# tomwhite/disq

Hardware: AMD Instinct MI355X
Metric: decompressed BAM GB/s + reads/sec (whole node) at 1/2/4/8 MI355X (higher is better)
Workload: dtype u8

## Files before the change

### disq_amd/csrc/dq_inflate3.hip

```cpp
#include "dq_inflate_core.h"
#include "dq_internal.h"

#include <mutex>
#include <vector>

namespace dq {
namespace {

using namespace dqi;

#define DQ_HD __device__ __host__ __attribute__((always_inline)) inline

#ifndef DQ_BLK_WG
#define DQ_BLK_WG 512
#endif
constexpr int WG = DQ_BLK_WG;
static_assert(WG % 128 == 0 && WG >= 512 && WG <= 1024, "whole waves on every SIMD");
constexpr int NWV = WG / 64;
constexpr int NDEC = WG;
constexpr uint32_t OV_DEFAULT = 96;
#ifndef DQ_TAIL_OV
#define DQ_TAIL_OV OV_DEFAULT
#endif
constexpr int OUTCAP = 65536 + 24;
#ifndef DQ_CSTEP
#define DQ_CSTEP 0
#endif
#ifndef DQ_RES_NB
#define DQ_RES_NB (WG == 512 ? 4 : 2)
#endif
#ifndef DQ_RES_G
#define DQ_RES_G 1
#endif
constexpr int RES_NXT = DQ_RES_NB * DQ_RES_G * WG;
constexpr int NCARRY = (65536 + RES_NXT - 1) / RES_NXT + 1;


constexpr int LR = 10, DR = 8;
constexpr int LSB = 15 - LR, DSB = 15 - DR;
constexpr int LSLOTS = 16, DSLOTS = 4;
constexpr int MAXGRP = 64;
constexpr int T_LSUB = 1 << LR;
constexpr int T_DROOT = T_LSUB + LSLOTS * (1 << LSB);
constexpr int T_DSUB = T_DROOT + (1 << DR);
constexpr int T_END = T_DSUB + DSLOTS * (1 << DSB);
constexpr int HB_WORDS = 160;
constexpr uint16_t E_SLOW = 0x0080;
constexpr uint32_t LL_EOB = 0xF810, LL_BAD = 0xF910;
DQ_HD uint16_t ent_ll(uint32_t sym, uint32_t len) {
  if (sym < 256) return (uint16_t)(sym << 8 | len);
  if (sym == 256) return (uint16_t)(LL_EOB | len);
  if (sym > 285) return (uint16_t)(LL_BAD | len);
  const uint32_t k = sym - 257;
  const uint32_t x = (k < 8 || k == 28) ? 0u : (k - 4) >> 2;
  const uint32_t base = k < 8 ? k + 3 : k == 28 ? 258u : ((4u + (k & 3u)) << ((k - 4) >> 2)) + 3u;
  return (uint16_t)((base - 3) << 8 | x << 5 | 16u | len);
}
DQ_HD uint16_t ent_d(uint32_t d, uint32_t len) {
  if (d >= 30) return (uint16_t)(0x4000u | len);
  const uint32_t x = d < 4 ? 0u : (d - 2) >> 1;
  const uint32_t m = d < 2 ? d : 2u + (d & 1u), sh = d < 2 ? 0u : (d >> 1) - 1u;
  return (uint16_t)(m << 12 | sh << 8 | x << 4 | len);
}

enum : int32_t { F_EXIT = 0, F_EOB = 1, F_ERR = 2, F_END = 3 };

constexpr int TOUT = 4096;
constexpr int TAIL_MAX_BITS = 32768;
constexpr int TW = 4;
#ifndef DQ_ROOT_REG
#define DQ_ROOT_REG 1
#endif
#ifndef DQ_TAIL_HDR1
#define DQ_TAIL_HDR1 1
#endif
constexpr int T_NCK = 4;
#ifndef DQ_TAIL_SEG
#define DQ_TAIL_SEG 96
#endif
constexpr int TAIL_SEG_MIN = DQ_TAIL_SEG;
constexpr int TIM_W = 32;
struct TailDesc {
  int32_t pos;
  int32_t produced;
  uint32_t crc_raw;
  int32_t flag;
};

struct alignas(16) LdsI {
  static constexpr int kLSUB = T_LSUB, kDROOT = T_DROOT, kDSUB = T_DSUB;
  [[maybe_unused]] static constexpr int kTEND = T_END;
  static constexpr bool kPair = true;
  alignas(8) uint32_t bm[2048];
  union {
    struct {
      uint16_t T[T_END];
      HuffCanon hl, hd;
      uint16_t lend[16], dend[16];
      uint16_t lent[288];
      uint16_t dent[32];
      union {
        uint16_t pair[1 << LR];
        struct {
          uint8_t lens[320];
          uint8_t clen[20];
          uint16_t clt[128];
          union {
            struct {
              int32_t cntw[NWV];
              int32_t cnts[NWV];
              uint32_t ginfo[MAXGRP + 32];
              uint32_t cntp[8][8];
              uint16_t pref[320];
            };
            struct {
              uint8_t exitm[NWV][16];
              int32_t ent[NWV + 1];
              int32_t wt[NWV];
              int32_t lv[NWV];
              int32_t endp;
            };
          };
        } h;
      } x;
    } d;
    struct {
      uint16_t last_start[1024];
      uint16_t nxt[RES_NXT];
      int32_t carry_ms[NCARRY];
      uint32_t carry_desc[NCARRY];
    } r;
    uint32_t crc4[4][256];
  } u;
  int32_t misc[32];
  union {
    struct {
      int32_t wsum[16];
      int32_t small[8 * 7];
    };
    uint32_t scratch[16 + 8 * 7];
  };
  alignas(16) uint8_t out[OUTCAP];
};
static_assert(sizeof(((LdsI*)nullptr)->scratch) >= 64 * 4, "one emit dummy word per lane");
static_assert(offsetof(LdsI, out) < 65536 - 4096, "the tables' offsets fit the DS offset field");
static_assert(2 * sizeof(LdsI) <= 160 * 1024, "two workgroups per CU");
static_assert(HB_WORDS * 4 <= T_END * 2, "header staging fits the decode table");

__device__ inline uint32_t* emit_dummy(LdsI& L) { return L.scratch; }

__constant__ uint32_t c_crc4[4][256];
__constant__ uint32_t c_x2n[32];
__constant__ uint32_t c_x8n[TOUT + 1];
constexpr int CRC_SL = 4 * (((65536 / 4 + WG - 1) / WG) | 1);
static_assert(CRC_SL * WG >= 65536, "the slices cover the largest block");
__constant__ uint32_t c_slice_shift[WG];
__constant__ uint8_t c_clorder3[19] = {16, 17, 18, 0, 8, 7, 9, 6, 10, 5, 11, 4, 12, 3, 13, 2, 14, 1, 15};

enum { M_ERR = 0, M_SLOW = 1 , M_A = 4, M_LAST, M_MORE, M_MORE1,
       M_LQ0 = 15, M_LQN, M_DQ0, M_DQN, M_NEXT,
       M_LASTF, M_RCNT = 28 ,
       M_DIRTY = 30  };

template <class LT>
__device__ __attribute__((always_inline)) inline void set_err(LT& L, int32_t code) { atomicCAS(&L.misc[M_ERR], 0, code); }


#define DQ_AI __device__ __attribute__((always_inline)) inline

DQ_AI int tid_fresh() {
  int t = (int)threadIdx.x;
  asm volatile("" : "+v"(t));
  return t;
}

typedef uint32_t u32x4 __attribute__((ext_vector_type(4)));
DQ_AI void st_nt(uint4* d, uint4 v) {
  u32x4 x = {v.x, v.y, v.z, v.w};
  __builtin_nontemporal_store(x, reinterpret_cast<u32x4*>(d));
}

struct GSrc {
  const uint32_t* __restrict__ p;
#ifdef DQ_CHECKED
  uint32_t lim;
  uint32_t tag;
#endif
  DQ_AI uint32_t operator[](uint32_t i) const {
#ifdef DQ_CHECKED
    DQ_CHKV(i < lim, CHK_K2_BITS, tag | min(i - lim + 1, 4095u));
#endif
    return *reinterpret_cast<const uint32_t*>(reinterpret_cast<const uint8_t*>(p) + (i << 2));
  }
};

#ifndef DQ_BR64
#define DQ_BR64 0
#endif
#if DQ_BR64
struct BitR {
  uint64_t bb;
  uint32_t bc;
  uint32_t wp;
  uint32_t nw;
};
template <class S>
DQ_AI void br_init(BitR& r, const S& W, uint32_t bitpos) {
  const uint32_t wi = bitpos >> 5;
  const uint64_t lo = W[wi], hi = W[wi + 1];
  const uint32_t sh = bitpos & 31;
  r.bb = ((hi << 32) | lo) >> sh;
  r.bc = 64 - sh;
  r.wp = wi + 2;
  r.nw = W[r.wp];
}
template <class S>
DQ_AI void br_refill(BitR& r, const S& W) {
  const bool need = r.bc <= 32;
  r.bb |= (uint64_t)(need ? r.nw : 0u) << r.bc;
  r.bc += need ? 32u : 0u;
  r.wp += need ? 1u : 0u;
  r.nw = W[r.wp];
}
DQ_AI uint32_t br_pos(const BitR& r) { return r.wp * 32 - r.bc; }
DQ_AI uint32_t br_peek(const BitR& r) { return (uint32_t)r.bb; }
template <class S>
DQ_AI void br_take(BitR& r, const S&, uint32_t n) {
  r.bb >>= n;
  r.bc -= n;
}
#else
struct BitR {
  uint32_t p;
  uint32_t w0, w1;
  uint32_t nw;
};
template <class S>
DQ_AI void br_init(BitR& r, const S& W, uint32_t bitpos) {
  const uint32_t wi = bitpos >> 5;
  r.w0 = W[wi];
  r.w1 = W[wi + 1];
  r.nw = W[wi + 2];
  r.p = bitpos;
}
template <class S>
DQ_AI void br_refill(BitR&, const S&) {}
DQ_AI uint32_t br_pos(const BitR& r) { return r.p; }
DQ_AI uint32_t br_peek(const BitR& r) { return __builtin_amdgcn_alignbit(r.w1, r.w0, r.p); }
template <class S>
DQ_AI void br_take(BitR& r, const S& W, uint32_t n) {
  const uint32_t q = r.p + n;
  const bool c = (q ^ r.p) >= 32u;
  r.w0 = c ? r.w1 : r.w0;
  r.w1 = c ? r.nw : r.w1;
  r.p = q;
  r.nw = W[(q >> 5) + 2];
}
#endif
DQ_AI uint32_t peek_bits(const uint32_t* __restrict__ W, uint32_t pos, uint32_t n) {
  const uint32_t wi = pos >> 5;
  const uint64_t v = ((uint64_t)W[wi + 1] << 32) | W[wi];
  return (uint32_t)(v >> (pos & 31)) & ((1u << n) - 1);
}

template <class LT>
DQ_AI uint32_t load_desc(const LT& L, int a) {
  const uint32_t* w = reinterpret_cast<const uint32_t*>(L.out + (a & ~3));
  return __builtin_amdgcn_alignbyte(w[1], w[0], (uint32_t)a & 3u) & 0xffffffu;
}

DQ_AI uint32_t zx16(uint16_t v) {
#ifndef DQ_NO_ZX16
  uint32_t x = v;
  asm("" : "+v"(x));
  return x;
#else
  return v;
#endif
}

template <bool SLOW, class LT>
DQ_AI uint32_t ll_second(const LT& L, uint32_t e, uint32_t bb) {
  const uint32_t sb = (e >> 4) & 7;
  DQ_CHK(LT::kLSUB + (e >> 7) + ((bb >> LR) & ((1u << sb) - 1)) < (uint32_t)LT::kDROOT, CHK_K2_TABLE);
  if (!SLOW) return L.u.d.T[LT::kLSUB + (e >> 7) + ((bb >> LR) & ((1u << sb) - 1))];
  if (sb) return L.u.d.T[LT::kLSUB + (e >> 7) + ((bb >> LR) & ((1u << sb) - 1))];
  if (!(e & E_SLOW)) return 0u;
  int l = 0;
  const int k = canon_decode(bb, L.u.d.hl, LR + 1, &l);
  return k < 0 ? 0u : L.u.d.lent[k];
}
template <bool SLOW, class LT>
DQ_AI uint32_t d_second(const LT& L, uint32_t e, uint32_t bb) {
  const uint32_t sb = (e >> 4) & 7;
  DQ_CHK(LT::kDSUB + (e >> 7) + ((bb >> DR) & ((1u << sb) - 1)) < (uint32_t)LT::kTEND, CHK_K2_TABLE);
  if (!SLOW) return L.u.d.T[LT::kDSUB + (e >> 7) + ((bb >> DR) & ((1u << sb) - 1))];
  if (sb) return L.u.d.T[LT::kDSUB + (e >> 7) + ((bb >> DR) & ((1u << sb) - 1))];
  if (!(e & E_SLOW)) return 0u;
  int l = 0;
  const int k = canon_decode(bb, L.u.d.hd, DR + 1, &l);
  return k < 0 ? 0u : L.u.d.dent[k];
}


template <bool SLOW, class S, class LT>
DQ_AI bool dsym(BitR& r, const S& W, const LT& L, uint32_t p, uint32_t lim,
                uint32_t& len, uint32_t& dist, uint32_t& lit2, bool& is_m, uint32_t& e) {
  br_refill(r, W);
  uint32_t bb = br_peek(r);
  const uint32_t ri = bb & ((1u << LR) - 1);
  e = L.u.d.T[ri];
  uint32_t pe = 0;
  if constexpr (LT::kPair) pe = zx16(L.u.d.x.pair[ri]);
  if ((e & 15) == 0) e = ll_second<SLOW>(L, e, bb);
  const uint32_t nb = e & 15;
  const uint32_t lx = __builtin_amdgcn_ubfe(e, 5, 3);
  is_m = (e & 16) != 0;
  len = (e >> 8) + (is_m ? 3u : 0u) + __builtin_amdgcn_ubfe(bb, nb, lx);
  const bool two = pe != 0 && p + nb < lim;
  lit2 = two ? pe >> 8 : 0xffffffffu;
  br_take(r, W, nb + lx + (two ? (pe & 15) : 0u));
  br_refill(r, W);
  bb = br_peek(r);
  uint32_t e2 = zx16(L.u.d.T[LT::kDROOT + (bb & ((1u << DR) - 1))]);
  if (is_m && (e2 & 15) == 0) e2 = d_second<SLOW>(L, e2, bb);
  const uint32_t nb2 = e2 & 15, dx = __builtin_amdgcn_ubfe(e2, 4, 4);
  dist = (__builtin_amdgcn_ubfe(e2, 12, 2) << __builtin_amdgcn_ubfe(e2, 8, 4)) + 1u +
         __builtin_amdgcn_ubfe(bb, nb2, dx);
  br_take(r, W, is_m ? nb2 + dx : 0u);
  return (SLOW && nb == 0) || (e & 0xFEF0u) == 0xF810u ||
         (is_m && ((SLOW && nb2 == 0) || (e2 & 0x4000u)));
}
DQ_AI uint32_t stop_end(uint32_t e, uint32_t p) {
  return (e & 15) != 0 && (e & 0xFFF0u) == LL_EOB ? p + (e & 15) : 0xffffffffu;
}
// ... 620 lines not shown
    const int32_t bfinal = (int32_t)(h & 1), btype = (int32_t)((h >> 1) & 3);
    const int32_t herr = pos + 3 > endbits ? ST_OVERREAD : btype == 3 ? ST_BAD_BLOCKTYPE : 0;
    if (herr) {
      if (t == 0) L.misc[M_ERR] = herr;
      break;
    }
    if (btype == 0) {
      const uint32_t q = (pos + 3 + 7) & ~7u;
      const uint8_t* bp = reinterpret_cast<const uint8_t*>(W) + q / 8;
      const uint32_t len = bp[0] | ((uint32_t)bp[1] << 8), nl = bp[2] | ((uint32_t)bp[3] << 8);
      const int32_t serr = (len ^ 0xffffu) != nl ? ST_BAD_STORED : q + 32 + 8 * len > endbits ? ST_OVERREAD : 0;
      if (serr) {
        if (t == 0) L.misc[M_ERR] = serr;
        break;
      }
      const uint8_t* sp = bp + 4;
      const int32_t n = min((int32_t)len, isize - produced);
      DQ_CHK(sh + produced + n <= OUTCAP, CHK_K2_IMAGE);
      for (int i = t; i < n; i += WG) L.out[sh + produced + i] = sp[i];
      produced += n;
      pos = q + 32 + 8 * len;
      __syncthreads();
      if (bfinal) break;
      continue;
    }
    const int nlen = btype == 1 ? 288 : (int)((h >> 3) & 31) + 257;
    const int ndist = btype == 1 ? 32 : (int)((h >> 8) & 31) + 1;
    if (btype == 2 && (nlen > 286 || ndist > 30)) {
      if (t == 0) L.misc[M_ERR] = ST_BAD_TABLE;
      break;
    }
    if (btype == 1) {
      for (int i = t; i < 320; i += WG) L.u.d.x.h.lens[i] = fixed_len(i);
      if (t == 0) L.misc[M_A] = (int32_t)(pos + 3);
      __syncthreads();
    } else {
      const int ncode = (int)((h >> 13) & 15) + 4;
      for (int i = t; i < 320; i += WG) L.u.d.x.h.lens[i] = 0;
      if (t < HB_WORDS) reinterpret_cast<uint32_t*>(L.u.d.T)[t] = hw;
      if (t < 19) L.u.d.x.h.clen[c_clorder3[t]] = t < ncode ? (uint8_t)hcl : 0;
      __syncthreads();
      if (t < 128) {
        bool ok = true;
        L.u.d.x.h.clt[t] = clt_entry(L.u.d.x.h.clen, t, &ok);
        if (t == 0 && !ok) set_err(L, ST_BAD_TABLE);
      }
      __syncthreads();
      if (L.misc[M_ERR]) break;
      {
        const uint64_t tr0 = TIMING ? __builtin_amdgcn_s_memtime() : 0;
        const uint32_t a = read_lengths(L, clpos + 3 * (uint32_t)ncode, nlen, ndist, endbits, hbase);
        if (t == 0) L.misc[M_A] = (int32_t)a;
        if (TIMING && t == 0) tacc[8] += __builtin_amdgcn_s_memtime() - tr0;
      }
      __syncthreads();
      if (L.misc[M_ERR]) break;
      if (L.u.d.x.h.lens[256] == 0) {
        if (t == 0) L.misc[M_ERR] = ST_BAD_TABLE;
        break;
      }
    }
    TST(0);
    build_tables(L, nlen, ndist);
    if (TIMING && t == 0) tacc[11] += __builtin_amdgcn_s_memtime() - tlast;
    if (L.misc[M_ERR]) break;
    for (int i = t; i < (1 << LR); i += WG) {
      const uint32_t e1 = L.u.d.T[i];
      const uint32_t l1 = e1 & 15;
      uint16_t v = 0;
      if (l1 > 0 && !(e1 & 16) && l1 < (uint32_t)LR) {
        const uint32_t e2 = L.u.d.T[(uint32_t)i >> l1];
        const uint32_t l2 = e2 & 15;
        if (l2 > 0 && !(e2 & 16) && l1 + l2 <= (uint32_t)LR)
          v = (uint16_t)e2;
      }
      L.u.d.x.pair[i] = v;
    }
    __syncthreads();
    TST(1);
    const uint32_t a = (uint32_t)L.misc[M_A];
    const bool slow = L.misc[M_SLOW] != 0;
    if (a > endbits) {
      if (t == 0) L.misc[M_ERR] = ST_OVERREAD;
      break;
    }
    const uint32_t span = endbits - a;
    const int ob = (sh + produced + 3) & ~3;
    const int cap = (sh + isize - ob) / (4 * (7 + NCK));
    int32_t* AB;
    int32_t* AE;
    int32_t* AC;
    int32_t* LS;
    int32_t* ST;
    int32_t* SE;
    int32_t* SC;
    uint32_t* CK = nullptr;
    const uint32_t maxl = (sflags >> 8) & 1023u, minseg = (sflags >> 20) & 1023u;
    int nl = (int)max(1u, min(maxl ? maxl : (uint32_t)NDEC, span / (minseg ? minseg : 128u)));
    nl = cap >= 8 ? min(nl, cap) : min(nl, 8);
    const uint32_t seg = (span + nl - 1) / nl;
    if (seg) nl = (int)((span + seg - 1) / seg);
    AB = cap >= 8 ? reinterpret_cast<int32_t*>(L.out + ob) : L.small;
    AE = AB + nl;
    AC = AE + nl;
    LS = AC + nl;
    ST = LS + nl;
    SE = ST + nl;
    SC = SE + nl;
    if (cap >= 8) CK = reinterpret_cast<uint32_t*>(SC + nl);
    DQ_CHK(cap < 8 || (ob >= sh + produced && ob + 4 * nl * (7 + NCK) <= OUTCAP), CHK_K2_LANES);
#ifdef DQ_CHECKED
    GSrc gsrc{W, (endbits >> 5) + 8, 1u << 12};
#else
    const GSrc gsrc{W};
#endif
    if (t == 0) {
      L.misc[M_RCNT] = 0;
      L.misc[M_LAST] = nl - 1;
    }
    if (t < nl) {
      const uint32_t sB = a + (uint32_t)t * seg;
      const uint32_t start = t == 0 ? a : (sB > a + OV ? sB - OV : a);
      const uint32_t sE = t == nl - 1 ? 0xffffffffu : a + (uint32_t)(t + 1) * seg;
      int32_t B = -1, E = 0, c = 0;
      if (CK)
        for (int j = 0; j < NCK; j++) CK[j * nl + t] = 0xffffffffu;
      const int f = slow ? run_seg<true>(gsrc, L, start, sB, sE, endbits, &B, &E, &c,
                                         CK ? CK + t : nullptr, nl, CKI, NCK)
                         : run_seg<false>(gsrc, L, start, sB, sE, endbits, &B, &E, &c,
                                          CK ? CK + t : nullptr, nl, CKI, NCK);
      AB[t] = B;
      AE[t] = (E << 3) | f;
      AC[t] = c;
      SE[t] = (E << 3) | f;
      SC[t] = c;
    }
    __syncthreads();
    TST(2);
#ifdef DQ_CHECKED
    gsrc.tag = 2u << 12;
#endif
    for (int round = 0; round <= nl; round++) {
      bool need = false;
      int32_t st = 0;
      if (t > 0 && t < nl) {
        const int32_t pe = AE[t - 1];
        st = pe >> 3;
        need = (pe & 7) == F_EXIT && AB[t] != st;
      }
      int32_t* rc = &L.misc[M_RCNT + (round & 1)];
      if (need) {
        const int r = atomicAdd(rc, 1);
        DQ_CHK(r < nl, CHK_K2_LANES);
        LS[r] = t;
        ST[r] = st;
      }
      if (t == 0) {
        L.misc[M_RCNT + ((round + 1) & 1)] = 0;
        L.misc[M_DIRTY + (round & 1)] = 0;
      }
      __syncthreads();
      const int nneed = *rc;
      if (nneed == 0) break;
      TCOUNT(10);
      const bool hi = __builtin_amdgcn_readfirstlane(t) < __builtin_amdgcn_readfirstlane(nneed);
      if (hi) __builtin_amdgcn_s_setprio(3);
      if (t < nneed) {
        const int lt = LS[t];
        const uint32_t s0 = (uint32_t)ST[t];
        const uint32_t sE = lt == nl - 1 ? 0xffffffffu : a + (uint32_t)(lt + 1) * seg;
        int32_t E = 0, c = 0;
        int jmerge = -1;
        const uint32_t sB = a + (uint32_t)lt * seg;
        const int f = slow ? run_redo<true>(gsrc, L, s0, sB, sE, endbits, CK ? CK + lt : nullptr,
                                            nl, SE[lt], SC[lt], &E, &c, CKI, NCK,
                                            TIMING ? &jmerge : nullptr)
                           : run_redo<false>(gsrc, L, s0, sB, sE, endbits, CK ? CK + lt : nullptr,
                                             nl, SE[lt], SC[lt], &E, &c, CKI, NCK,
                                             TIMING ? &jmerge : nullptr);
        const int32_t ae = (E << 3) | f;
        if (ae != AE[lt]) L.misc[M_DIRTY + (round & 1)] = 1;
        AB[lt] = (int32_t)s0;
        AE[lt] = ae;
        AC[lt] = c;
        if (TIMING) {
          atomicAdd(&L.misc[21], 1);
          if (jmerge >= 0) {
            atomicAdd(&L.misc[23], 1);
            atomicAdd(&L.misc[24], jmerge);
          } else {
            const int sf = SE[lt] & 7;
            atomicAdd(&L.misc[sf == F_ERR || sf == F_EOB ? 25 : sf == F_EXIT ? 26 : 27], 1);
          }
        }
      }
      if (hi) __builtin_amdgcn_s_setprio(0);
      __syncthreads();
      if (L.misc[M_DIRTY + (round & 1)] == 0) break;
    }
    TST(3);

    int32_t myB = 0, myE = 0, myF = F_DEAD, myC = 0;
    if (t < nl) {
      myB = AB[t];
      myE = AE[t] >> 3;
      myF = AE[t] & 7;
      myC = AC[t];
    }
    if (t < nl && myF != F_EXIT) atomicMin(&L.misc[M_LAST], t);
    __syncthreads();
    const int last = L.misc[M_LAST];
    const int32_t cv = t <= last ? myC : 0;
    const int32_t incl = wave_incl_scan(cv, lane);
    if (lane == 63) L.wsum[wv] = incl;
    if (t == last) {
      L.misc[M_NEXT] = myE;
      L.misc[M_LASTF] = myF;
    }
    __syncthreads();
    int32_t woff = 0;
    for (int w = 0; w < wv; w++) woff += L.wsum[w];
    const int32_t myoff = produced + woff + incl - cv;
    int32_t total = 0;
    for (int w = 0; w < WG / 64; w++) total += L.wsum[w];
    const bool full = produced + total >= isize;
    const int32_t fl = L.misc[M_LASTF];
    if (!full && fl != F_EOB && t == 0) L.misc[M_ERR] = fl == F_ERR ? ST_BAD_CODE : ST_SHORT;
    __syncthreads();
    TST(4);
    if (L.misc[M_ERR]) break;
#ifdef DQ_CHECKED
    gsrc.tag = 3u << 12;
#endif
    if (t <= last && myoff < isize) {
      const uint32_t sE = t == nl - 1 ? 0xffffffffu : a + (uint32_t)(t + 1) * seg;
      if (slow) emit_seg<true>(gsrc, L, (uint32_t)myB, sE, endbits, myoff, isize, sh);
      else emit_seg<false>(gsrc, L, (uint32_t)myB, sE, endbits, myoff, isize, sh);
    }
    const int32_t nextpos = L.misc[M_NEXT];
    __syncthreads();
    TST(5);
    produced = min(isize, produced + total);
    if (TIMING && t == 0) {
      if (tacc[22] == 0)
        for (int i = 0; i < 6; i++) tacc[16 + i] = tacc[i];
      tacc[22] += 1;
    }
    if (full || bfinal) break;
    pos = (uint32_t)nextpos;
    if (tails && isize - produced <= TOUT && endbits - pos <= (uint32_t)TAIL_MAX_BITS) {
      deferred = true;
      break;
    }
  }
  __syncthreads();
  int32_t err = L.misc[M_ERR];
  if (!err && !deferred && produced != isize) err = ST_SHORT;
  const int32_t rsize = deferred ? produced : isize;
  if (deferred && t == 0) {
    TailDesc td;
    td.pos = (int32_t)pos;
    td.produced = produced;
    td.crc_raw = 0;
    td.flag = 1;
    tails[blockIdx.x] = td;
  }
  if (err) {
    if (t == 0) status[b] = err;
    return;
  }
  const uint64_t* bm64 = reinterpret_cast<const uint64_t*>(L.bm);
  {
    int ls[2];
    int run = -1;
#pragma unroll
    for (int k = 0; k < 2; k++) {
      const uint64_t m = 2 * t + k < 1024 ? bm64[min(2 * t + k, 1023)] : 0ull;
      if (m) run = 64 * (2 * t + k) + 63 - __clzll(m);
      ls[k] = run;
    }
    const int wm = wave_incl_max(run);
    if (lane == 63) L.wsum[wv] = wm;
    int ex = __shfl_up(wm, 1, 64);
    if (lane == 0) ex = -1;
    __syncthreads();
    for (int w = 0; w < wv; w++) ex = max(ex, L.wsum[w]);
#pragma unroll
    for (int k = 0; k < 2; k++) {
      const int v = max(ex, ls[k]);
      if (WG == 512 || 2 * t + k < 1024) L.u.r.last_start[2 * t + k] = v < 0 ? (uint16_t)0xffff : (uint16_t)v;
    }
    __syncthreads();
  }
  uint8_t* dstU = U + ub;
  const uint8_t* O = L.out + sh;
  const int head = min((16 - sh) & 15, rsize);
  int32_t lines_done = 0;
  constexpr int CH = G * WG;
  constexpr int BATCH = NB * CH;
  constexpr int NE = NB * G;
  constexpr bool CSTEP = (DQ_CSTEP != 0 && G > 1) || CH % 512 != 0;
  static_assert(BATCH <= RES_NXT, "the batch's next-pointers fit the resolve scratch");
  static_assert((65536 + BATCH - 1) / BATCH <= NCARRY, "one carry slot per batch");
  uint16_t* nxt = L.u.r.nxt;
  auto first_hop = [&](int32_t b0, int32_t cms, uint32_t cdesc, int32_t* fr, int32_t* xs,
                       bool& pending) {
    pending = false;
    uint64_t mw[NB];
    int32_t lsv[NB];
#pragma unroll
    for (int k = 0; k < NB; k++) {
      const int32_t g0 = b0 + k * CH + G * t;
      const int w = min(g0 >> 6, 1023);
      DQ_CHK(w >= 0 && w - 1 < 1024, CHK_K2_LAST);
      mw[k] = bm64[w];
      lsv[k] = w ? (int32_t)zx16(L.u.r.last_start[w - 1]) : 0xffff;
    }
    int32_t msv[NE];
    uint32_t da[NB], db[NB];
#pragma unroll
    for (int k = 0; k < NB; k++) {
      const int32_t g0 = b0 + k * CH + G * t;
#pragma unroll
      for (int i = 0; i < G; i++) {
        const uint64_t mi = mw[k] & (~0ull >> (63 - ((g0 + i) & 63)));
        msv[k * G + i] = mi ? (g0 | 63) - (int32_t)__clzll(mi) : lsv[k];
      }
      da[k] = load_desc(L, sh + min(msv[k * G], 65535));
      db[k] = G > 1 ? load_desc(L, sh + min(msv[k * G + G - 1], 65535)) : da[k];
    }
#pragma unroll
    for (int k = 0; k < NB; k++) {
      const int32_t g0 = b0 + k * CH + G * t;
      const int32_t sbk = b0 + k * CH + (CSTEP ? 0 : ((G * t) & ~511));
#pragma unroll
      for (int i = 0; i < G; i++) {
        const int e = k * G + i;
        const int32_t x = g0 + i, ms = msv[e];
        const bool before = ms < b0;
        const uint32_t desc = before ? cdesc : (ms == msv[k * G + G - 1] ? db[k] : da[k]);
        const int32_t len = (int32_t)(desc >> 15) + 3, D1 = (int32_t)(desc & 0x7fff);
        const bool copy = x < rsize && ms != 0xffff && (!before || ms == cms) && x < ms + len;
        const int32_t jj = x - ms;
        int32_t src = (int32_t)((uint32_t)D1 ^ ~0u) + x;
        if (__builtin_expect(__any(copy && jj > D1), 0)) {
          const int32_t D = D1 + 1;
          const int32_t q = (int32_t)((float)jj * __builtin_amdgcn_rcpf((float)D));
          int32_t r = jj - q * D;
          r = r >= D ? r - D : r;
          src = ms - D + r;
        }
        DQ_CHK(!copy || (src >= 0 && src < x), CHK_K2_SRC);
        const bool done = !copy || src < sbk;
        fr[e] = copy ? src : x;
        xs[e] = done ? x : src;
        pending = pending || !done;
        nxt[x - b0] = (uint16_t)(copy ? src : x);
      }
    }
  };
  auto jump_round = [&](int32_t b0, int32_t* fr, int32_t* xs, bool& pending) {
    int32_t qv[NE];
#pragma unroll
    for (int e = 0; e < NE; e++) {
      DQ_CHK(xs[e] - b0 >= 0 && xs[e] - b0 < BATCH, CHK_K2_NXT);
      qv[e] = (int32_t)zx16(nxt[xs[e] - b0]);
    }
    bool any = false;
#pragma unroll
    for (int e = 0; e < NE; e++) {
      const int32_t own = (e / G) * CH + G * t + e % G;
      const int32_t p = xs[e], q = qv[e];
      const bool pd = p != b0 + own;
      const int32_t sbk = b0 + (e / G) * CH + (CSTEP ? 0 : ((G * t) & ~511));
      const bool fin = pd && (q == p || q < sbk);
      const bool go = pd && !fin;
      fr[e] = fin ? q : fr[e];
      xs[e] = go ? q : b0 + own;
      any = any || go;
      nxt[own] = (uint16_t)q;
    }
    pending = any;
  };
  int32_t frA[NE], xsA[NE];
  bool pendA = false;
  int32_t cms = -1;
  uint32_t cdesc = 0;
  first_hop(0, cms, cdesc, frA, xsA, pendA);
  if (t < (rsize + BATCH - 1) / BATCH) {
    int32_t ncms = -1;
    uint32_t ncdesc = 0;
    const int32_t x = (t + 1) * BATCH - 1;
    if (x + 1 < rsize) {
      const uint64_t m = bm64[x >> 6];
      const int32_t ms = m ? (x | 63) - (int32_t)__clzll(m) : (int32_t)L.u.r.last_start[(x >> 6) - 1];
      if (ms != 0xffff) {
        const uint32_t desc = load_desc(L, sh + ms);
        if (ms + (int32_t)(desc >> 15) + 3 > x + 1) {
          ncms = ms;
          ncdesc = desc;
        }
      }
    }
    L.u.r.carry_ms[t] = ncms;
    L.u.r.carry_desc[t] = ncdesc;
  }
  __syncthreads();
  for (int hop = 0; pendA && hop < WG + 2; hop++) jump_round(0, frA, xsA, pendA);
  for (int32_t bs = 0; bs < rsize; bs += BATCH) {
    const uint64_t tb0 = TIMING ? __builtin_amdgcn_s_memtime() : 0;
    const int32_t nbs = bs + BATCH;
    const bool more = nbs < rsize;
    __syncthreads();
    const int32_t ncms = more ? L.u.r.carry_ms[bs / BATCH] : -1;
    const uint32_t ncdesc = more ? L.u.r.carry_desc[bs / BATCH] : 0u;
    int32_t frB[NE], xsB[NE];
    bool pendB = false;
    if (more) first_hop(nbs, ncms, ncdesc, frB, xsB, pendB);
    const uint64_t tb1 = TIMING ? __builtin_amdgcn_s_memtime() : 0;
#pragma unroll
    for (int k = 0; k < NB; k++) {
#pragma unroll
      for (int j = 0; j < (CSTEP ? 1 : G); j++) {
        const bool mine = CSTEP || ((G * t) >> 9) == j;
        const int32_t g0 = bs + k * CH + G * t;
        uint8_t v[G];
        if (mine)
#pragma unroll
          for (int i = 0; i < G; i++) {
            DQ_CHK(g0 + i >= rsize || (frA[k * G + i] >= 0 && frA[k * G + i] <= g0 + i), CHK_K2_SRC);
            v[i] = O[min(frA[k * G + i], 65535)];
          }
        if ((k > 0 || j > 0) && pendB) jump_round(nbs, frB, xsB, pendB);
        if (mine)
#pragma unroll
          for (int i = 0; i < G; i++)
            if (g0 + i < rsize) L.out[sh + g0 + i] = v[i];
        __syncthreads();
      }
    }
    if (pendB) jump_round(nbs, frB, xsB, pendB);
    const uint64_t tb2 = TIMING ? __builtin_amdgcn_s_memtime() : 0;
    const int32_t c1 = min(rsize, nbs);
    const int32_t lines_to = c1 >= head ? (c1 - head) / 16 : 0;
    if (!(sflags & 1)) {
      for (int32_t k = lines_done + t; k < lines_to; k += WG) {
        const uint4 v = *reinterpret_cast<const uint4*>(O + head + 16 * k);
        uint4* d = reinterpret_cast<uint4*>(dstU + head + 16 * k);
        if (sflags & 2) st_nt(d, v);
        else *d = v;
      }
      lines_done = lines_to;
    }
    const uint64_t tb3 = TIMING ? __builtin_amdgcn_s_memtime() : 0;
    for (int hop = 0; pendB && hop < WG + 2; hop++) jump_round(nbs, frB, xsB, pendB);
#pragma unroll
    for (int e = 0; e < NE; e++) frA[e] = frB[e];
    cms = ncms;
    cdesc = ncdesc;
    if (TIMING && t == 0) {
      tacc[9] += tb1 - tb0;
      tacc[12] += tb2 - tb1;
      tacc[13] += tb3 - tb2;
      tacc[14] += __builtin_amdgcn_s_memtime() - tb3;
      tacc[15] += 1;
    }
  }
  if (sflags & 1) {
    const int32_t lines_to = rsize >= head ? (rsize - head) / 16 : 0;
    for (int32_t k = t; k < lines_to; k += WG) {
      const uint4 v = *reinterpret_cast<const uint4*>(O + head + 16 * k);
      uint4* d = reinterpret_cast<uint4*>(dstU + head + 16 * k);
      if (sflags & 2) st_nt(d, v);
      else *d = v;
    }
    lines_done = lines_to;
  }
  uint32_t ct0 = 0, ct1 = 0, cshift = 0, cinit = 0, cwant = 0;
  if (verify_crc) {
    ct0 = (&c_crc4[0][0])[t];
    ct1 = t + WG < 1024 ? (&c_crc4[0][0])[t + WG] : 0u;
    cshift = c_slice_shift[WG - 1 - t];
    if (t == 0) {
      cinit = crc_init[rsize];
      const uint8_t* tr = C + cpos + csize - 8;
      cwant = (uint32_t)tr[0] | ((uint32_t)tr[1] << 8) | ((uint32_t)tr[2] << 16) | ((uint32_t)tr[3] << 24);
    }
  }
  static_assert(2 * WG >= 1024, "at most two CRC table words per thread");
  for (int x = t; x < head; x += WG) dstU[x] = O[x];
  for (int x = head + 16 * lines_done + t; x < rsize; x += WG) dstU[x] = O[x];
  TST(6);
  if (verify_crc) {
    __syncthreads();
    if (t < 1024) (&L.u.crc4[0][0])[t] = ct0;
    if (t + WG < 1024) (&L.u.crc4[0][0])[t + WG] = ct1;
    __syncthreads();
    const int32_t e = rsize - (WG - 1 - t) * CRC_SL;
    const int32_t s0 = max(0, e - CRC_SL);
    uint32_t cr = 0;
    if (e > 0) {
      int32_t x = s0;
      while (x < e && ((sh + x) & 3)) cr = L.u.crc4[0][(cr ^ O[x++]) & 0xff] ^ (cr >> 8);
      for (; x + 4 <= e; x += 4) {
        const uint32_t v = cr ^ *reinterpret_cast<const uint32_t*>(O + x);
        cr = L.u.crc4[3][v & 0xff] ^ L.u.crc4[2][(v >> 8) & 0xff] ^ L.u.crc4[1][(v >> 16) & 0xff] ^
             L.u.crc4[0][v >> 24];
      }
      while (x < e) cr = L.u.crc4[0][(cr ^ O[x++]) & 0xff] ^ (cr >> 8);
      cr = gf2_mulmod(cshift, cr);
    }
    cr = wave_incl_xor(cr);
    if (lane == 63) L.wsum[wv] = (int32_t)cr;
    __syncthreads();
    if (t == 0) {
      uint32_t x = 0;
      for (int w = 0; w < WG / 64; w++) x ^= (uint32_t)L.wsum[w];
      if (deferred) {
        tails[blockIdx.x].crc_raw = x;
      } else {
        const uint32_t crc = (x ^ cinit) ^ 0xffffffffu;
        if (crc != cwant) status[b] = ST_CRC;
      }
    }
  }
  TST(7);
  if (TIMING && t == 0)
    for (int i = 0; i < 24; i++) tim[(int64_t)blockIdx.x * TIM_W + i] = tacc[i];
  if (TIMING && t == 0)
    for (int i = 0; i < 7; i++) tim[(int64_t)blockIdx.x * TIM_W + 24 + i] = (uint64_t)L.misc[21 + i];
}

struct alignas(16) LdsW {
  static constexpr int kLSUB = 0, kDROOT = 1 << LR, kDSUB = 0, kTEND = (1 << LR) + (1 << DR);
  static constexpr bool kPair = false;
  union {
    struct {
      uint16_t T[kTEND];
      HuffCanon hl, hd;
      uint16_t lend[16], dend[16];
      uint16_t lent[288];
      uint16_t dent[32];
      union {
        struct {
          uint8_t lens[320];
          uint8_t clen[20];
          uint16_t clt[128];
          int32_t cnt[32];
          int32_t run[32];
        } h;
      } x;
    } d;
    uint32_t crc4[4][256];
  } u;
  alignas(16) uint8_t out[TOUT + 32];
  alignas(8) uint32_t bm[TOUT / 32];
  uint32_t ck[T_NCK * 64];
  int32_t misc[8];
  uint32_t scratch[16];
};
static_assert(HB_WORDS * 4 <= LdsW::kTEND * 2, "header staging fits the decode table");
static_assert(4 * 4 * sizeof(LdsW) <= 160 * 1024, "four tails per workgroup, four workgroups per CU");
DQ_AI uint32_t* emit_dummy(LdsW& L) { return L.ck; }

DQ_AI uint32_t read_lengths_wave(LdsW& L, uint32_t P, int nlen, int ndist, uint32_t endbits,
                                 uint32_t hbase) {
  const uint32_t* hb = reinterpret_cast<const uint32_t*>(L.u.d.T);
  auto& H = L.u.d.x.h;
  const int lane = tid_fresh() & 63;
  const int total = nlen + ndist;
  int have = 0, prev = -1, entry = 0;
  for (uint32_t W0 = P;; W0 += 64) {
    if (W0 > endbits) {
      set_err(L, ST_OVERREAD);
      return W0;
    }
    const uint32_t p = W0 + (uint32_t)lane;
    const uint32_t wi = min((p >> 5) - hbase, (uint32_t)HB_WORDS - 2);
    const uint32_t v = (uint32_t)((((uint64_t)hb[wi + 1] << 32) | hb[wi]) >> (p & 31));
    const uint32_t ent = H.clt[v & 127];
    const uint32_t cl = ent & 7, sy = ent >> 3;
    const uint32_t ex = sy == 16 ? 2u : sy == 17 ? 3u : sy == 18 ? 7u : 0u;
    const int xv = (int)((v >> cl) & ((1u << ex) - 1));
    const int rep = sy < 16 ? 1 : sy == 16 ? 3 + xv : sy == 17 ? 3 + xv : 11 + xv;
    const int adv = cl ? (int)(cl + ex) : 0;
    int J[6];
    J[0] = adv ? min(lane + adv, 64) : lane;
#pragma unroll
    for (int k = 1; k < 6; k++) {
      const int y = __shfl(J[k - 1], J[k - 1] & 63, 64);
      J[k] = J[k - 1] >= 64 ? 64 : y;
    }
    int pk = entry;
#pragma unroll
    for (int k = 0; k < 6; k++) {
      const int y = __shfl(J[k], pk & 63, 64);
      if ((lane >> k) & 1) pk = pk >= 64 ? 64 : y;
    }
    const bool onp = pk < 64;
    const int src = pk & 63;
    const int s_rep = __shfl(rep, src, 64), s_adv = __shfl(adv, src, 64);
    const int s_sy = __shfl((int)sy, src, 64);
    const int pprev = __shfl_up(pk, 1, 64);
    const bool real = onp && (lane == 0 || pprev != pk);
    const bool bad = real && s_adv == 0;
    const int r = real && !bad ? s_rep : 0;
    const int incl = wave_incl_scan(r, lane);
    const int key = wave_incl_max(real && !bad && s_sy != 16 ? ((lane + 1) << 5) | (s_sy < 16 ? s_sy : 0) : 0);
    const int kprev = __shfl_up(key, 1, 64);
    const int before = lane == 0 ? 0 : kprev;
    const int val = s_sy < 16 ? s_sy : s_sy == 16 ? (before > 0 ? (before & 31) : prev) : 0;
    const bool take = real && have + incl - r < total;
    if (__any((take && bad) || (take && s_sy == 16 && val < 0) || (take && have + incl > total))) {
      set_err(L, ST_BAD_TABLE);
      return W0;
    }
    if (take && val != 0)
      for (int i = have + incl - r; i < have + incl; i++) H.lens[i < nlen ? i : 288 + i - nlen] = (uint8_t)val;
    const uint64_t tk = __ballot(take);
    const int lastk = tk ? 63 - (int)__clzll(tk) : -1;
    if (lastk >= 0 && __shfl(have + incl, lastk, 64) >= total) {
      __builtin_amdgcn_wave_barrier();
      return W0 + (uint32_t)__shfl(pk + s_adv, lastk, 64);
    }
    const uint64_t rm = __ballot(real);
    const int lastr = rm ? 63 - (int)__clzll(rm) : -1;
    if (lastr < 0 || __shfl((int)bad, lastr, 64)) {
      set_err(L, ST_BAD_TABLE);
      return W0;
    }
    have = __shfl(have + incl, lastr, 64);
    const int kl = __shfl(key, 63, 64);
    prev = kl > 0 ? (kl & 31) : prev;
    entry = __shfl(pk + s_adv, lastr, 64) - 64;
  }
}

DQ_AI void build_tables_wave(LdsW& L, int nlen, int ndist) {
  const int lane = tid_fresh() & 63;
  auto& H = L.u.d.x.h;
  if (lane < 32) {
    H.cnt[lane] = 0;
    H.run[lane] = 0;
  }
  __builtin_amdgcn_wave_barrier();
  for (int k = lane; k < 320; k += 64) {
    const bool isl = k < 288;
    const int len = isl ? (k < nlen ? H.lens[k] : 0) : (k - 288 < ndist ? H.lens[k] : 0);
    if (len) atomicAdd(&H.cnt[(isl ? 0 : 16) + len], 1);
  }
  __builtin_amdgcn_wave_barrier();
  __builtin_amdgcn_fence(__ATOMIC_SEQ_CST, "wavefront");
  int e = 0;
  {
    const int l = lane & 15;
    const bool in = lane < 32 && l >= 1;
    const int c = in ? H.cnt[lane] : 0;
    int offi = wave_incl_scan(c, lane);
    const int tt = in ? c << (16 - l) : 0;
    int cs = wave_incl_scan(tt, lane);
    const int base_o = __shfl(offi, 15, 64), base_c = __shfl(cs, 15, 64);
    if (lane >= 16) {
      offi -= base_o;
      cs -= base_c;
    }
    const int code = in ? (int)((uint32_t)(cs - tt) >> (16 - l)) : 0;
    const int left = in ? (1 << l) - (code + c) : 0;
    const bool isd = lane >= 16;
    HuffCanon& h = isd ? L.u.d.hd : L.u.d.hl;
    uint16_t* end = isd ? L.u.d.dend : L.u.d.lend;
    const int R = isd ? DR : LR;
    if (lane < 32) {
      h.first[l] = (uint16_t)code;
      h.count[l] = (uint16_t)c;
      h.offs[l] = (uint16_t)(offi - c);
      if (in && l <= R) end[l] = (uint16_t)((code + c) << (R - l));
    }
    const uint64_t over = __ballot(in && left < 0);
    const uint64_t used = __ballot(c > 0);
    const int left15l = __shfl(left, 15, 64), left15d = __shfl(left, 31, 64);
    const uint64_t ul = used & 0xffffull, ud = (used >> 16) & 0xffffull;
    const int maxll = ul ? 63 - __clzll(ul) : 0, maxld = ud ? 63 - __clzll(ud) : 0;
    if (over) e = ST_BAD_TABLE;
    if (maxll > 0 && left15l > 0 && maxll != 1) e = ST_BAD_TABLE;
    if (maxld > 0 && left15d > 0 && maxld != 1) e = ST_BAD_TABLE;
    const int ql0 = __shfl(offi, LR, 64), qln = __shfl(offi, 15, 64);
    const int qd0 = __shfl(offi, 16 + DR, 64), qdn = __shfl(offi, 31, 64);
    if (lane == 0) L.misc[M_SLOW] = (qln > ql0 || qdn > qd0) ? 1 : 0;
  }
  if (e) {
    if (lane == 0) set_err(L, e);
    return;
  }
  __builtin_amdgcn_wave_barrier();
  const uint64_t below = lanes_below(lane);
  for (int k0 = 0; k0 < 320; k0 += 64) {
    const int k = k0 + lane;
    const bool isl = k < 288;
    const int sym = isl ? k : k - 288;
    const int len = k < 320 ? (isl ? (k < nlen ? H.lens[k] : 0) : (sym < ndist ? H.lens[k] : 0)) : 0;
    const int key = (isl ? 0 : 16) + len;
    uint64_t peers = ~0ull;
#pragma unroll
    for (int bt = 0; bt < 5; bt++) {
      const uint64_t bl = __ballot((key >> bt) & 1);
      peers &= ((key >> bt) & 1) ? bl : ~bl;
    }
    const int run0 = H.run[key];
    const int rank = run0 + __popcll(peers & below);
    __builtin_amdgcn_wave_barrier();
    if (len && (peers >> lane) == 1ull) H.run[key] = run0 + __popcll(peers);
    if (len) {
      const HuffCanon& hh = isl ? L.u.d.hl : L.u.d.hd;
      const int q = hh.offs[len] + rank;
      if (isl) L.u.d.lent[q] = ent_ll((uint32_t)sym, (uint32_t)len);
      else L.u.d.dent[q] = ent_d((uint32_t)sym, (uint32_t)len);
    }
    __builtin_amdgcn_wave_barrier();
  }
  __builtin_amdgcn_wave_barrier();
  const bool lslow = L.u.d.hl.count[11] + L.u.d.hl.count[12] + L.u.d.hl.count[13] +
                         L.u.d.hl.count[14] + L.u.d.hl.count[15] > 0;
  const bool dslow = L.u.d.hd.count[9] + L.u.d.hd.count[10] + L.u.d.hd.count[11] + L.u.d.hd.count[12] +
                         L.u.d.hd.count[13] + L.u.d.hd.count[14] + L.u.d.hd.count[15] > 0;
#if DQ_ROOT_REG
  const RootEnds<LR> le = root_ends<LR>(L.u.d.lend);
  const RootEnds<DR> de = root_ends<DR>(L.u.d.dend);
#endif
  for (int i = lane; i < (1 << LR); i += 64) {
#if DQ_ROOT_REG
    const uint16_t v = root_entry_r<LR>(L.u.d.hl, le, L.u.d.lent, bitrev((uint32_t)i, LR));
#else
    const uint16_t v = root_entry<LR>(L, L.u.d.hl, L.u.d.lend, L.u.d.lent, bitrev((uint32_t)i, LR));
#endif
    L.u.d.T[i] = v ? v : lslow ? E_SLOW : (uint16_t)(LL_BAD | 1u);
  }
  for (int i = lane; i < (1 << DR); i += 64) {
#if DQ_ROOT_REG
    const uint16_t v = root_entry_r<DR>(L.u.d.hd, de, L.u.d.dent, bitrev((uint32_t)i, DR));
#else
// ... 553 lines not shown
```

Baseline: 179.9.

## Resolve back-reference pointers four at a time with packed LDS stores

```diff
diff --git a/disq_amd/csrc/dq_inflate3.hip b/disq_amd/csrc/dq_inflate3.hip
--- a/disq_amd/csrc/dq_inflate3.hip
+++ b/disq_amd/csrc/dq_inflate3.hip
@@ -31,6 +31,9 @@
 #endif
 #ifndef DQ_RES_G
 #define DQ_RES_G 1
+#endif
+#ifndef DQ_RES_QUAD
+#define DQ_RES_QUAD 1
 #endif
 constexpr int RES_NXT = DQ_RES_NB * DQ_RES_G * WG;
 constexpr int NCARRY = (65536 + RES_NXT - 1) / RES_NXT + 1;
@@ -1257,10 +1260,79 @@
   constexpr bool CSTEP = (DQ_CSTEP != 0 && G > 1) || CH % 512 != 0;
   static_assert(BATCH <= RES_NXT, "the batch's next-pointers fit the resolve scratch");
   static_assert((65536 + BATCH - 1) / BATCH <= NCARRY, "one carry slot per batch");
+  static_assert(CSTEP || CH / 512 <= G, "the G ordered steps of a chunk cover it");
+  constexpr bool QUAD = G == 4 && DQ_RES_QUAD != 0;
+  constexpr bool HYB = G == 1 && NB == 4 && WG == 512 && !CSTEP && DQ_RES_QUAD != 0;
+  constexpr int GK = HYB ? 1 : NB, GCH = HYB ? BATCH : CH;
+  static_assert(!(QUAD || HYB) || offsetof(LdsI, u.r.nxt) % 8 == 0, "a group's next pointers are one 64-bit word");
+  constexpr bool INR = 65536 % BATCH == 0;
   uint16_t* nxt = L.u.r.nxt;
+  auto pack16 = [](int32_t lo, int32_t hi) {
+    return __builtin_amdgcn_perm((uint32_t)hi, (uint32_t)lo, 0x05040100u);
+  };
+  auto med3 = [](int32_t a, int32_t b, int32_t c) { return max(min(a, b), min(max(a, b), c)); };
+  auto store_nxt4 = [&](int off, uint32_t lo, uint32_t hi) {
+    const uint2 v = make_uint2(lo, hi);
+    __builtin_memcpy(__builtin_assume_aligned(nxt + off, 8), &v, 8);
+  };
   auto first_hop = [&](int32_t b0, int32_t cms, uint32_t cdesc, int32_t* fr, int32_t* xs,
                        bool& pending) {
     pending = false;
+    if constexpr (QUAD || HYB) {
+#pragma unroll
+      for (int k = 0; k < GK; k++) {
+        const int32_t g0 = b0 + k * GCH + 4 * t;
+        const int w = INR ? g0 >> 6 : min(g0 >> 6, 1023);
+        DQ_CHK(w >= 0 && w < 1024, CHK_K2_LAST);
+        const uint64_t m = bm64[w];
+        const int32_t ls = w ? (int32_t)zx16(L.u.r.last_start[w - 1]) : 0xffff;
+        const uint32_t bit = (uint32_t)g0 & 60u;
+        const uint64_t below = m & ~(~0ull << bit);
+        const int32_t prev = below ? (g0 | 63) - (int32_t)__clzll(below) : ls;
+        const uint32_t nib = (uint32_t)(m >> bit) & 15u;
+        DQ_CHK(g0 >= rsize || ((0x0317u >> nib) & 1u), CHK_K2_BM);
+        const bool hasB = nib != 0;
+        const int32_t A = (nib & 1u) ? g0 : prev;
+        const int32_t Bs = hasB ? g0 + 31 - (int32_t)__clz(nib) : A;
+        const uint32_t ldA = load_desc(L, sh + (INR ? A : min(A, 65535)));
+        const uint32_t ldB = load_desc(L, sh + (INR ? Bs : min(Bs, 65535)));
+        const uint32_t dA = A < b0 ? cdesc : ldA;
+        const uint32_t dB = hasB ? ldB : dA;
+        const int32_t D1A = (int32_t)(dA & 0x7fff), D1B = (int32_t)(dB & 0x7fff);
+        const int32_t remA = A == 0xffff ? 0 : rsize - A;
+        const int32_t limA = med3(remA, 0, (int32_t)(dA >> 15) + 3);
+        const int32_t limB = med3(hasB ? rsize - Bs : remA, 0, (int32_t)(dB >> 15) + 3);
+        const int32_t sbk = b0 + k * GCH + (CSTEP ? 0 : ((4 * t) & ~511));
+        int32_t f4[4];
+#pragma unroll
+        for (int i = 0; i < 4; i++) {
+          const int32_t x = g0 + i;
+          const bool useB = i == 0 ? false : i == 3 ? true : x >= Bs;
+          const int32_t ms = useB ? Bs : A, lim = useB ? limB : limA, D1 = useB ? D1B : D1A;
+          const int32_t jj = x - ms;
+          const bool copy = (uint32_t)jj < (uint32_t)lim;
+          int32_t src = (int32_t)((uint32_t)D1 ^ ~0u) + x;
+          if (__builtin_expect(__any(copy && jj > D1), 0)) {
+            const int32_t D = D1 + 1;
+            const int32_t q = (int32_t)((float)jj * __builtin_amdgcn_rcpf((float)D));
+            int32_t r = jj - q * D;
+            r = r >= D ? r - D : r;
+            src = ms - D + r;
+          }
+          DQ_CHK(!copy || (src >= 0 && src < x), CHK_K2_SRC);
+          f4[i] = copy ? src : x;
+          if constexpr (QUAD) {
+            const bool done = !copy || src < sbk;
+            fr[4 * k + i] = f4[i];
+            xs[4 * k + i] = done ? x : src;
+            pending = pending || !done;
+          }
+        }
+        DQ_CHK(k * GCH + 4 * t + 3 < BATCH, CHK_K2_NXT);
+        store_nxt4(k * GCH + 4 * t, pack16(f4[0], f4[1]), pack16(f4[2], f4[3]));
+      }
+      return;
+    }
     uint64_t mw[NB];
     int32_t lsv[NB];
 #pragma unroll
@@ -1314,6 +1386,22 @@
       }
     }
   };
+  auto adopt = [&](int32_t b0, int32_t* fr, int32_t* xs, bool& pending) {
+    int32_t qv[NE];
+#pragma unroll
+    for (int e = 0; e < NE; e++) qv[e] = (int32_t)zx16(nxt[(e / G) * CH + G * t + e % G]);
+    pending = false;
+#pragma unroll
+    for (int e = 0; e < NE; e++) {
+      const int32_t x = b0 + (e / G) * CH + G * t + e % G;
+      const int32_t sbk = b0 + (e / G) * CH + ((G * t) & ~511);
+      const int32_t q = qv[e];
+      const bool done = q == x || q < sbk;
+      fr[e] = q;
+      xs[e] = done ? x : q;
+      pending = pending || !done;
+    }
+  };
   auto jump_round = [&](int32_t b0, int32_t* fr, int32_t* xs, bool& pending) {
     int32_t qv[NE];
 #pragma unroll
@@ -1333,7 +1421,12 @@
       fr[e] = fin ? q : fr[e];
       xs[e] = go ? q : b0 + own;
       any = any || go;
-      nxt[own] = (uint16_t)q;
+      if constexpr (!QUAD) nxt[own] = (uint16_t)q;
+    }
+    if constexpr (QUAD) {
+#pragma unroll
+      for (int k = 0; k < NB; k++)
+        store_nxt4(k * CH + 4 * t, pack16(qv[4 * k], qv[4 * k + 1]), pack16(qv[4 * k + 2], qv[4 * k + 3]));
     }
     pending = any;
   };
@@ -1361,6 +1454,7 @@
     L.u.r.carry_desc[t] = ncdesc;
   }
   __syncthreads();
+  if constexpr (HYB) adopt(0, frA, xsA, pendA);
   for (int hop = 0; pendA && hop < WG + 2; hop++) jump_round(0, frA, xsA, pendA);
   for (int32_t bs = 0; bs < rsize; bs += BATCH) {
     const uint64_t tb0 = TIMING ? __builtin_amdgcn_s_memtime() : 0;
@@ -1384,13 +1478,36 @@
 #pragma unroll
           for (int i = 0; i < G; i++) {
             DQ_CHK(g0 + i >= rsize || (frA[k * G + i] >= 0 && frA[k * G + i] <= g0 + i), CHK_K2_SRC);
-            v[i] = O[min(frA[k * G + i], 65535)];
+            v[i] = O[INR ? frA[k * G + i] : min(frA[k * G + i], 65535)];
           }
+        if constexpr (HYB)
+          if (k == 1 && more) adopt(nbs, frB, xsB, pendB);
         if ((k > 0 || j > 0) && pendB) jump_round(nbs, frB, xsB, pendB);
-        if (mine)
-#pragma unroll
-          for (int i = 0; i < G; i++)
-            if (g0 + i < rsize) L.out[sh + g0 + i] = v[i];
+        if constexpr (QUAD && INR) {
+          if (mine) {
+            const uint32_t lo = (uint32_t)v[0] | (uint32_t)v[1] << 8;
+            const uint32_t hi = (uint32_t)v[2] | (uint32_t)v[3] << 8;
+            uint8_t* const p = L.out + sh + g0;
+            if ((sh & 3) == 0) {
+              const uint32_t w4 = lo | hi << 16;
+              __builtin_memcpy(__builtin_assume_aligned(p, 4), &w4, 4);
+            } else if ((sh & 3) == 2) {
+              const uint16_t a2 = (uint16_t)lo, b2 = (uint16_t)hi;
+              __builtin_memcpy(__builtin_assume_aligned(p, 2), &a2, 2);
+              __builtin_memcpy(__builtin_assume_aligned(p + 2, 2), &b2, 2);
+            } else {
+              const uint16_t m2 = (uint16_t)(v[1] | v[2] << 8);
+              p[0] = v[0];
+              __builtin_memcpy(__builtin_assume_aligned(p + 1, 2), &m2, 2);
+              p[3] = v[3];
+            }
+          }
+        } else {
+          if (mine)
+#pragma unroll
+            for (int i = 0; i < G; i++)
+              if (g0 + i < rsize) L.out[sh + g0 + i] = v[i];
+        }
         __syncthreads();
       }
     }
```

After: 185.7, median of 6. +3.2%, better.
